# NVlabs/latentfusion

Hardware: AMD Instinct MI355X
Metric: pose-optim iters/sec (reconstruct+render+backward), 16 views, 128^3 voxels (higher is better)
Workload: dtype f32

## Files before the change

latentfusion_amd/csrc/build.py:

```python
import os
import subprocess
import sys

HERE = os.path.dirname(os.path.abspath(__file__))
SOURCES = ['resample.hip', 'splat.hip', 'conv.hip', 'pointwise.hip', 'image.hip', 'optim.hip', 'resize.hip', 'conv_split.hip', 'conv_wino.hip', 'wgrad.hip', 'sample2d.hip', 'gru.hip', 'wino_gemm.hip', 'reduce.hip', 'wino_fused.hip', 'conv_bf16.hip', 'occlusion.hip', 'conv_gru.hip', 'lift_mfma.hip', 'pw16.hip', 'wino_fused_f16x3.hip', 'wgrad_wide.hip', 'rows_gemm.hip', 'ibr.hip', 'latent.hip', 'points.hip', 'depth_init.hip', 'obs_prepare.hip', 'train_loss.hip', 'depth_points.hip', 'fps.hip']
LIB = os.path.join(HERE, 'liblf_hip.so')
EXTRA = {'conv_split.hip': ['-fno-slp-vectorize'], 'conv_gru.hip': ['-fno-slp-vectorize']}
FLAGS = ['--offload-arch=gfx950', '-O3', '-std=c++17', '-fPIC', '-fno-gpu-rdc', '-Wall', '-Wno-unused-function']


def _hipcc():
    for cand in (os.environ.get('HIPCC'), '/opt/rocm/bin/hipcc', 'hipcc'):
        if cand and (os.path.isabs(cand) and os.path.exists(cand) or not os.path.isabs(cand)):
            return cand
    raise RuntimeError('hipcc not found')


def needs_build():
    if not os.path.exists(LIB):
        return True
    t = os.path.getmtime(LIB)
    deps = [os.path.join(HERE, s) for s in SOURCES if os.path.exists(os.path.join(HERE, s))]
    deps += [os.path.join(HERE, f) for f in os.listdir(HERE) if f.endswith(('.h', '.inc'))]
    deps += [os.path.join(HERE, '..', '..', 'include', 'lf_hip.h'), os.path.join(HERE, '..', '..', 'include', 'lf_hip_experimental.h')]
    return any(os.path.getmtime(d) > t for d in deps)


def build(force=False, verbose=True):
    if not force and not needs_build():
        return LIB
    hipcc = _hipcc()
    objs = []
    procs = []
    for src in SOURCES:
        path = os.path.join(HERE, src)
        if not os.path.exists(path):
            continue
        obj = os.path.join(HERE, src.replace('.hip', '.o'))
        objs.append(obj)
        cmd = [hipcc, '-x', 'hip', '-c', path, '-o', obj] + FLAGS + EXTRA.get(src, [])
        procs.append((cmd, subprocess.Popen(cmd, stdout=subprocess.PIPE, stderr=subprocess.STDOUT)))
    for cmd, p in procs:
        out, _ = p.communicate()
        if p.returncode != 0:
            raise RuntimeError('hipcc failed: ' + ' '.join(cmd) + '\n' + out.decode())
        if verbose and out.strip():
            print(out.decode())
    cmd = [hipcc, '-shared', '-fPIC', '--offload-arch=gfx950', '-o', LIB] + objs
    r = subprocess.run(cmd, stdout=subprocess.PIPE, stderr=subprocess.STDOUT)
    if r.returncode != 0:
        raise RuntimeError('link failed:\n' + r.stdout.decode())
    if verbose:
        print('built', LIB)
    return LIB


if __name__ == '__main__':
    build(force='--force' in sys.argv)
```

latentfusion_amd/csrc/conv.hip:

```cpp
#include "lf_common.h"

namespace {

constexpr int TX = 16;

template <int DIMS> struct TileGeom;
template <> struct TileGeom<3> { static constexpr int TY = 4, TZ = 4, HY = 6, HZ = 6, TAPS = 27; };
template <> struct TileGeom<2> { static constexpr int TY = 16, TZ = 1, HY = 18, HZ = 1, TAPS = 9; };

template <int NT, int NR, bool WHOLE = false>
__device__ __forceinline__ void epilogue_store(f32x4 (&acc)[NT][NR], const long (&rowoff)[NR], const long (&rowidx)[NR],
                                               const float* __restrict__ bias, float* __restrict__ y,
                                               float* __restrict__ norm_out, int Cout, int co_base,
                                               int ysc, long yss, bool vec_out,
                                               float he, unsigned flags, float slope, float eps,
                                               const float* __restrict__ prev_y = nullptr,
                                               const float* __restrict__ prev_norm = nullptr, unsigned prev_flags = 0,
                                               float* __restrict__ amax_out = nullptr) {
  float lane_amax = 0.f;
  const int lane = threadIdx.x & 63;
  const int cq = lane >> 4;
  float bv[NT][4];
#pragma unroll
  for (int t = 0; t < NT; ++t)
// ... 619 lines not shown
  if (c16 <= 32) return 32;
  return (c16 + 63) & ~63;
}

extern "C" int lf_conv1x1_cout_padded(int Cout) {
  lf_clear_error();
  const int c16 = (Cout + 15) & ~15;
  if (c16 <= 16) return 16;
  if (c16 <= 32) return 32;
  if (c16 <= 64) return 64;
  return (c16 + 127) & ~127;
}

static int conv3x3_launch(const float* x, const float* wpack, const float* bias, float* y, float* norm_out,
                          int dims, int N, int D, int H, int W, int Cin, int Cout,
                          float he, unsigned flags, float slope, float eps, void* stream,
                          const float* prev_y, const float* prev_norm, unsigned prev_flags) {
  if (N <= 0 || D <= 0 || H <= 0 || W <= 0 || Cin <= 0 || Cout <= 0) return LF_EINVAL;
  if (prev_y != nullptr) {
    if (flags != 0 || bias != nullptr || (Cout != 16 && Cout != 32 && Cout != 64) || !lf_aligned16(prev_y)) return LF_EINVAL;
    if ((prev_flags & LF_EPI_PIXELNORM) && prev_norm == nullptr) return LF_EINVAL;
  }
  if (dims != 2 && dims != 3) return LF_EINVAL;
  if (dims == 2 && D != 1) return LF_EINVAL;
  if ((flags & LF_EPI_PIXELNORM) && Cout > 64) return LF_EINVAL;
  if (!lf_aligned16(x) || !lf_aligned16(y) || !lf_aligned16(wpack)) return LF_EALIGN;
  const int CinP = (Cin + 15) & ~15, CoutP = lf_conv3x3_cout_padded(Cout);
  const int ntiles = CoutP / 16;
  const int NT = ntiles >= 4 ? 4 : ntiles;
  const int groups = ntiles / NT;
  const int TY = dims == 3 ? 4 : 16, TZ = dims == 3 ? 4 : 1;
  const int tiles_x = (W + TX - 1) / TX, tiles_y = (H + TY - 1) / TY, tiles_z = (D + TZ - 1) / TZ;
  const long nblk = (long)tiles_x * tiles_y * tiles_z * N;
  if (nblk > 0x7fffffffL) return LF_EINVAL;
  dim3 grid((unsigned)nblk, groups), block(256);
  hipStream_t s = (hipStream_t)stream;
  if (Cin == 16 && Cout == 16 && dims == 3 && (long)D * H * W >= 4096 && (long)D * H * W * 64 < 0x7fffffffL &&
      slope > 0.f && slope < 1.f && (bias == nullptr || lf_aligned16(bias))) {
    const int ptx = (W + TX - 1) / TX, pty = (H + p3::TY - 1) / p3::TY, ptz = (D + p3::TZ - 1) / p3::TZ;
    const long pt = (long)ptx * pty * ptz * N;
    if (pt <= 0x7fffffffL) {
      const int cus = lf_cu_count();
      const unsigned pgrid = (unsigned)(pt < cus ? pt : cus);
      hipLaunchKernelGGL(conv3d_c16_persistent_kernel, dim3(pgrid), dim3(p3::NTHREADS), 0, s, x, wpack, bias, y, norm_out,
                         N, D, H, W, ptx, pty, ptz, (int)pt, he, flags, slope, eps, prev_y, prev_norm, prev_flags);
      return lf_launch_status();
    }
  }
  if (CinP == 16 && CoutP == 16) {
    if (dims == 3)
      hipLaunchKernelGGL((conv3x3_c16_kernel<3>), grid, block, 0, s, x, wpack, bias, y, norm_out, N, D, H, W, Cin, Cout,
                         tiles_x, tiles_y, tiles_z, he, flags, slope, eps, prev_y, prev_norm, prev_flags);
    else
      hipLaunchKernelGGL((conv3x3_c16_kernel<2>), grid, block, 0, s, x, wpack, bias, y, norm_out, N, D, H, W, Cin, Cout,
                         tiles_x, tiles_y, tiles_z, he, flags, slope, eps, prev_y, prev_norm, prev_flags);
    return lf_launch_status();
  }
#define LAUNCH(DM, T) hipLaunchKernelGGL((conv3x3_kernel<DM, T>), grid, block, 0, s, x, wpack, bias, y, norm_out, \
                                         N, D, H, W, Cin, Cout, CinP, CoutP, tiles_x, tiles_y, tiles_z, he, flags, slope, eps, \
                                         prev_y, prev_norm, prev_flags)
  if (dims == 3) { if (NT == 4) LAUNCH(3, 4); else if (NT == 2) LAUNCH(3, 2); else LAUNCH(3, 1); }
  else           { if (NT == 4) LAUNCH(2, 4); else if (NT == 2) LAUNCH(2, 2); else LAUNCH(2, 1); }
#undef LAUNCH
  return lf_launch_status();
}

extern "C" int lf_conv3x3_fwd(const float* x, const float* wpack, const float* bias, float* y, float* norm_out,
                              int dims, int N, int D, int H, int W, int Cin, int Cout,
                              float he, unsigned flags, float slope, float eps, void* stream) {
  lf_clear_error();
  return conv3x3_launch(x, wpack, bias, y, norm_out, dims, N, D, H, W, Cin, Cout, he, flags, slope, eps, stream,
                        nullptr, nullptr, 0);
}

extern "C" int lf_conv3x3_bwd_data(const float* gy, const float* wpack_t, float* gx, int dims, int N, int D, int H, int W,
                                   int Cin, int Cout, float he, const float* prev_y, const float* prev_norm,
                                   unsigned prev_flags, float slope, void* stream) {
  lf_clear_error();
  return conv3x3_launch(gy, wpack_t, nullptr, gx, nullptr, dims, N, D, H, W, Cin, Cout, he, 0, slope, 0.f, stream,
                        prev_y, prev_norm, prev_flags);
}

static int conv1x1_launch(const float* x, const float* wpack, const float* bias, float* y, float* norm_out,
                          int N, int P, int Cin, int ksl, long x_batch_stride, long x_slice_stride,
                          int Cout, long y_batch_stride, int y_row_stride, int y_slice_channels,
                          long y_slice_stride,
                          float he, unsigned flags, float slope, float eps, void* stream,
                          const float* prev_y, const float* prev_norm, unsigned prev_flags, float* amax_out = nullptr,
                          const float* xscale = nullptr) {
  if (N <= 0 || P <= 0 || Cin <= 0 || ksl <= 0 || Cout <= 0 || y_slice_channels <= 0) return LF_EINVAL;
  if (xscale != nullptr && (Cin & 3)) return LF_EALIGN;
  if (prev_y != nullptr) {
    if (flags != 0 || bias != nullptr || y_slice_channels != 16 || y_row_stride != 16 || (Cout & 15) ||
        !lf_aligned16(prev_y) || ((y_batch_stride | y_slice_stride) & 15))
      return LF_EINVAL;
    if ((prev_flags & LF_EPI_PIXELNORM) && prev_norm == nullptr) return LF_EINVAL;
    if ((prev_flags & LF_EPI_DOT) && (prev_flags != LF_EPI_DOT || prev_norm == nullptr)) return LF_EINVAL;
  }
  if (y_row_stride < (y_slice_channels < Cout ? y_slice_channels : Cout)) return LF_EINVAL;
  if (ksl > 1 && (Cin & 3)) return LF_EALIGN;
  if ((flags & LF_EPI_PIXELNORM) && Cout > 128) return LF_EINVAL;
  if (!lf_aligned16(x) || !lf_aligned16(y) || !lf_aligned16(wpack)) return LF_EALIGN;
  if (y == nullptr && !(prev_y != nullptr && (prev_flags & LF_EPI_DOT))) return LF_EINVAL;
  if ((Cin & 3) == 0 && ((x_batch_stride | x_slice_stride) & 3)) return LF_EALIGN;
  const int K = ksl * Cin, Kp = (K + 15) & ~15;
  const int CoutP = lf_conv1x1_cout_padded(Cout);
  const int ntiles = CoutP / 16;
  const int NT = ntiles >= 8 ? ((prev_y != nullptr && ntiles >= 16) ? 4 : 8) : ntiles;
  const int groups = ntiles / NT;
  dim3 grid((unsigned)((P + 63) / 64), groups, N), block(256);
  hipStream_t s = (hipStream_t)stream;
#define LAUNCH(T) hipLaunchKernelGGL((conv1x1_kernel<T>), grid, block, 0, s, x, wpack, bias, y, norm_out, \
                                     P, Cin, ksl, x_batch_stride, x_slice_stride, Cout, Kp, y_batch_stride, y_row_stride, \
                                     y_slice_channels, y_slice_stride, he, flags, slope, eps, prev_y, prev_norm, prev_flags, \
                                     amax_out, xscale)
  switch (NT) {
    case 1: LAUNCH(1); break;
    case 2: LAUNCH(2); break;
    case 4: LAUNCH(4); break;
    case 8: LAUNCH(8); break;
    default: return LF_EINVAL;
  }
#undef LAUNCH
  return lf_launch_status();
}

extern "C" int lf_conv1x1_fwd(const float* x, const float* wpack, const float* bias, float* y, float* norm_out,
                              int N, int P, int Cin, int ksl, long x_batch_stride, long x_slice_stride,
                              int Cout, long y_batch_stride, int y_row_stride, int y_slice_channels,
                              long y_slice_stride,
                              float he, unsigned flags, float slope, float eps, void* stream) {
  lf_clear_error();
  return conv1x1_launch(x, wpack, bias, y, norm_out, N, P, Cin, ksl, x_batch_stride, x_slice_stride, Cout,
                        y_batch_stride, y_row_stride, y_slice_channels, y_slice_stride, he, flags, slope, eps, stream,
                        nullptr, nullptr, 0);
}

extern "C" int lf_conv1x1_fwd_scaled(const float* x, const float* xscale, const float* wpack, const float* bias, float* y,
                                     float* norm_out, int N, int P, int Cin, int ksl, long x_batch_stride, long x_slice_stride,
                                     int Cout, long y_batch_stride, int y_row_stride, int y_slice_channels, long y_slice_stride,
                                     float he, unsigned flags, float slope, float eps, void* stream) {
  lf_clear_error();
  if (xscale == nullptr) return LF_EINVAL;
  return conv1x1_launch(x, wpack, bias, y, norm_out, N, P, Cin, ksl, x_batch_stride, x_slice_stride, Cout,
                        y_batch_stride, y_row_stride, y_slice_channels, y_slice_stride, he, flags, slope, eps, stream,
                        nullptr, nullptr, 0, nullptr, xscale);
}

extern "C" int lf_conv1x1_bwd_data(const float* gy, const float* wpack_t, float* gx, int N, int P, int Cin, int Cout,
                                   long y_batch_stride, int y_row_stride, int y_slice_channels, long y_slice_stride,
                                   float he, const float* prev_y, const float* prev_norm, unsigned prev_flags,
                                   float slope, float* amax_out, void* stream) {
  lf_clear_error();
  return conv1x1_launch(gy, wpack_t, nullptr, gx, nullptr, N, P, Cin, 1, (long)P * Cin, 0, Cout, y_batch_stride,
                        y_row_stride, y_slice_channels, y_slice_stride, he, 0, slope, 0.f, stream, prev_y, prev_norm,
                        prev_flags, amax_out);
}
```

latentfusion_amd/csrc/conv_wino.hip:

```cpp
#include "wino16_compute.h"

namespace {

template <bool SPLIT, int FUSE = 0, bool PACK = false, int FORM = WF_GENERIC, int OPT = 0, int ZST = 0>
__device__ __forceinline__ void conv3d_c16_wino_body(
    const float* __restrict__ x, const float* __restrict__ upack, const float* __restrict__ bias,
    float* __restrict__ y, float* __restrict__ norm_out,
    int N, int D, int H, int W, int tiles_x, int tiles_y, int tiles_z, int ntiles,
    float he, unsigned flags, float slope, float eps,
    const float* __restrict__ prev_y, const float* __restrict__ prev_norm, unsigned prev_flags,
    const float* __restrict__ amax_in, float* __restrict__ amax_out, const WinoProj pj = WinoProj()) {
  static_assert(FORM == WF_GENERIC || (!SPLIT && FUSE != 2 && PACK), "fixed forms: the packed all-fp32 kernels only");
  static_assert(OPT == 0 || OPT == 1, "");
  static_assert(FORM != WF_GENERIC || OPT == 0, "the generic kernel stays as it is");
  static_assert(ZST == 0 || (ZST == 1 && FORM != WF_GENERIC), "z-staged halo: the fixed forms only");
  constexpr bool HAS_BIAS = FORM == WF_FWD_BLOCK;
  if constexpr (FORM == WF_FWD_BLOCK) {
    flags = LF_EPI_LRELU | LF_EPI_PIXELNORM;
    prev_y = nullptr; prev_norm = nullptr; prev_flags = 0u; amax_out = nullptr;
  } else if constexpr (FORM == WF_DGRAD_PREV) {
    flags = 0u; prev_flags = LF_EPI_LRELU | LF_EPI_PIXELNORM;
    bias = nullptr; norm_out = nullptr; amax_out = nullptr;
  } else if constexpr (FORM == WF_DGRAD_PLAIN) {
    flags = 0u; prev_flags = 0u;
// ... 255 lines not shown
        v[k] = wino_epi_dgrad_plain(o[k], out_scale);
      } else if (prev_y == nullptr || addmode) {
        float ss = 0.f;
#pragma unroll
        for (int e = 0; e < 4; ++e) {
          float u = o[k][e] * out_scale + bv4[e];
          if (addmode) u += pyv[k][e];
          if (flags & LF_EPI_LRELU) u = fmaxf(u, u * slope);
          v[k][e] = u;
          ss += u * u;
        }
        if (flags & LF_EPI_PIXELNORM) {
          const float tq = quad_sum(ss) * (1.f / 16.f) + eps;
          const float rinv = fast_rsqrt(tq);
          rn[k] = tq * rinv;
          v[k] *= rinv;
        }
      }
    }
    TS(6);
    if constexpr (FUSE != 2) halo_commit();
    TS(7);
#pragma unroll
    for (int k = 0; k < 4; ++k) {
      if constexpr (FORM == WF_DGRAD_PREV) {
        if (!(WINO_ABL & 1)) v[k] = wino_epi_dgrad_prev(o[k], pyv[k], pnv[k], out_scale, slope);
      } else if (!(WINO_ABL & 1) && prev_y != nullptr && !addmode) {
        const f32x4 yp = pyv[k];
        v[k] = o[k] * out_scale;
        if (prev_flags & LF_EPI_PIXELNORM) {
          const float dot = quad_sum(v[k][0] * yp[0] + v[k][1] * yp[1] + v[k][2] * yp[2] + v[k][3] * yp[3]) * (1.f / 16.f);
          const float rinv = fast_rcp(pnv[k]);
#pragma unroll
          for (int e = 0; e < 4; ++e) v[k][e] = (v[k][e] - yp[e] * dot) * rinv;
        }
        if (prev_flags & LF_EPI_LRELU) {
#pragma unroll
          for (int e = 0; e < 4; ++e) v[k][e] = yp[e] > 0.f ? v[k][e] : v[k][e] * slope;
        }
      }
      if (okv[k]) {
        __builtin_nontemporal_store(v[k], (f32x4*)(ybase + (unsigned)(voxi[k] * 64)));
        if (!(WINO_ABL & 16) && (prev_y == nullptr || addmode) && (flags & LF_EPI_PIXELNORM) && (FORM == WF_FWD_BLOCK || nbase != nullptr) && eq == 0) nbase[voxi[k]] = rn[k];
        if (amax_out != nullptr)
          wave_amax = fmaxf(wave_amax, fmaxf(fmaxf(fabsf(v[k][0]), fabsf(v[k][1])), fmaxf(fabsf(v[k][2]), fabsf(v[k][3]))));
      }
    }
    if constexpr (FUSE == 2) {
#define WINO16_PROJBWD_NEXT
#include "wino16_projbwd.inc"
    }
    if constexpr (FUSE == 1) {
#define WINO16_PROJFWD_TILE
#include "wino16_projfwd.inc"
    }
    TS(8);
    lds_barrier();
    cx = nx; cy = ny; cz = nz; cn = nn;
    if constexpr (FUSE == 2) {
#define WINO16_PROJBWD_COLUMN
#include "wino16_projbwd.inc"
    }
  }
  if (amax_out != nullptr) {
    float m = wave_amax;
#pragma unroll
    for (int o2 = 32; o2 > 0; o2 >>= 1) m = fmaxf(m, __shfl_xor(m, o2, 64));
    lf_amax_publish(amax_out, m, lane);
  }
}

template <bool PACK>
__global__ void __launch_bounds__(256, 2) conv3d_c16_wino_kernel(
    const float* __restrict__ x, const float* __restrict__ upack, const float* __restrict__ bias,
    float* __restrict__ y, float* __restrict__ norm_out, int N, int D, int H, int W, int tiles_x, int tiles_y, int tiles_z,
    int ntiles, float he, unsigned flags, float slope, float eps, const float* __restrict__ prev_y,
    const float* __restrict__ prev_norm, unsigned prev_flags, float* __restrict__ amax_out) {
  conv3d_c16_wino_body<false, 0, PACK>(x, upack, bias, y, norm_out, N, D, H, W, tiles_x, tiles_y, tiles_z, ntiles, he, flags, slope, eps,
                              prev_y, prev_norm, prev_flags, nullptr, amax_out);
}

__global__ void __launch_bounds__(256, 2) conv3d_c16_wino_f16x3_kernel(
    const float* __restrict__ x, const float* __restrict__ upack, const float* __restrict__ bias,
    float* __restrict__ y, float* __restrict__ norm_out, int N, int D, int H, int W, int tiles_x, int tiles_y, int tiles_z,
    int ntiles, float he, unsigned flags, float slope, float eps, const float* __restrict__ prev_y,
    const float* __restrict__ prev_norm, unsigned prev_flags, const float* __restrict__ amax_in,
    float* __restrict__ amax_out) {
  conv3d_c16_wino_body<true>(x, upack, bias, y, norm_out, N, D, H, W, tiles_x, tiles_y, tiles_z, ntiles, he, flags, slope, eps,
                             prev_y, prev_norm, prev_flags, amax_in, amax_out);
}

template <bool PACK>
__global__ void __launch_bounds__(256, 2) conv3d_c16_wino_projfwd_kernel(
    const float* __restrict__ x, const float* __restrict__ upack, const float* __restrict__ bias,
    float* __restrict__ y, float* __restrict__ norm_out, int N, int D, int H, int W, int tiles_x, int tiles_y, int tiles_z,
    int ntiles, float he, unsigned flags, float slope, float eps, const float* __restrict__ prev_y,
    const float* __restrict__ prev_norm, unsigned prev_flags, WinoProj pj) {
  conv3d_c16_wino_body<false, 1, PACK>(x, upack, bias, y, norm_out, N, D, H, W, tiles_x, tiles_y, tiles_z, ntiles, he, flags, slope,
                                 eps, prev_y, prev_norm, prev_flags, nullptr, nullptr, pj);
}

template <bool PACK>
__global__ void __launch_bounds__(256, 2) conv3d_c16_wino_projbwd_kernel(
    const float* __restrict__ x, const float* __restrict__ upack, const float* __restrict__ bias,
    float* __restrict__ y, float* __restrict__ norm_out, int N, int D, int H, int W, int tiles_x, int tiles_y, int tiles_z,
    int ntiles, float he, unsigned flags, float slope, float eps, const float* __restrict__ prev_y,
    const float* __restrict__ prev_norm, unsigned prev_flags, WinoProj pj) {
  conv3d_c16_wino_body<false, 2, PACK>(x, upack, bias, y, norm_out, N, D, H, W, tiles_x, tiles_y, tiles_z, ntiles, he, flags, slope,
                                 eps, prev_y, prev_norm, prev_flags, nullptr, nullptr, pj);
}

template <int FORM, int OPT>
__global__ void __launch_bounds__(256, 2) conv3d_c16_wino_form_kernel(
    const float* __restrict__ x, const float* __restrict__ upack, const float* __restrict__ bias,
    float* __restrict__ y, float* __restrict__ norm_out, int N, int D, int H, int W, int tiles_x, int tiles_y, int tiles_z,
    int ntiles, float he, unsigned flags, float slope, float eps, const float* __restrict__ prev_y,
    const float* __restrict__ prev_norm, unsigned prev_flags, float* __restrict__ amax_out) {
  conv3d_c16_wino_body<false, 0, true, FORM, OPT>(x, upack, bias, y, norm_out, N, D, H, W, tiles_x, tiles_y, tiles_z, ntiles, he, flags,
                                                 slope, eps, prev_y, prev_norm, prev_flags, nullptr, amax_out);
}

template <int FORM, int OPT>
__global__ void __launch_bounds__(256, 2) conv3d_c16_wino_projfwd_form_kernel(
    const float* __restrict__ x, const float* __restrict__ upack, const float* __restrict__ bias,
    float* __restrict__ y, float* __restrict__ norm_out, int N, int D, int H, int W, int tiles_x, int tiles_y, int tiles_z,
    int ntiles, float he, unsigned flags, float slope, float eps, const float* __restrict__ prev_y,
    const float* __restrict__ prev_norm, unsigned prev_flags, WinoProj pj) {
  conv3d_c16_wino_body<false, 1, true, FORM, OPT>(x, upack, bias, y, norm_out, N, D, H, W, tiles_x, tiles_y, tiles_z, ntiles, he, flags,
                                                 slope, eps, prev_y, prev_norm, prev_flags, nullptr, nullptr, pj);
}

template <int FORM, int OPT>
__global__ void __launch_bounds__(256, 2) conv3d_c16_wino_zst_form_kernel(
    const float* __restrict__ x, const float* __restrict__ upack, const float* __restrict__ bias,
    float* __restrict__ y, float* __restrict__ norm_out, int N, int D, int H, int W, int tiles_x, int tiles_y, int tiles_z,
    int ntiles, float he, unsigned flags, float slope, float eps, const float* __restrict__ prev_y,
    const float* __restrict__ prev_norm, unsigned prev_flags, float* __restrict__ amax_out) {
  conv3d_c16_wino_body<false, 0, true, FORM, OPT, 1>(x, upack, bias, y, norm_out, N, D, H, W, tiles_x, tiles_y, tiles_z, ntiles, he, flags,
                                                    slope, eps, prev_y, prev_norm, prev_flags, nullptr, amax_out);
}

template <int FORM, int OPT>
__global__ void __launch_bounds__(256, 2) conv3d_c16_wino_projfwd_zst_form_kernel(
    const float* __restrict__ x, const float* __restrict__ upack, const float* __restrict__ bias,
    float* __restrict__ y, float* __restrict__ norm_out, int N, int D, int H, int W, int tiles_x, int tiles_y, int tiles_z,
    int ntiles, float he, unsigned flags, float slope, float eps, const float* __restrict__ prev_y,
    const float* __restrict__ prev_norm, unsigned prev_flags, WinoProj pj) {
  conv3d_c16_wino_body<false, 1, true, FORM, OPT, 1>(x, upack, bias, y, norm_out, N, D, H, W, tiles_x, tiles_y, tiles_z, ntiles, he, flags,
                                                    slope, eps, prev_y, prev_norm, prev_flags, nullptr, nullptr, pj);
}

int g_wino_pack = 1;
int g_wino_forms = 1;
constexpr bool wino_zst_default[4] = {true, false, false, true};
bool wino_zst(int idx) { return g_wino_forms == 4 || (g_wino_forms == 1 && wino_zst_default[idx]); }

int wino_form_of(const float* bias, const float* norm_out, unsigned flags, const float* prev_y, const float* prev_norm,
                 unsigned prev_flags, const float* amax_out) {
  const unsigned full = LF_EPI_LRELU | LF_EPI_PIXELNORM;
  if (!g_wino_pack || !g_wino_forms || amax_out != nullptr) return WF_GENERIC;
  if (flags == full && bias != nullptr && norm_out != nullptr && prev_y == nullptr) return WF_FWD_BLOCK;
  if (flags == 0u && bias == nullptr && prev_y != nullptr && prev_norm != nullptr && prev_flags == full) return WF_DGRAD_PREV;
  if (flags == 0u && bias == nullptr && prev_y == nullptr) return WF_DGRAD_PLAIN;
  return WF_GENERIC;
}

template <auto kernel, bool COLUMNS = false, typename... Extra>
int launch_wino(const float* x, const void* upack, const float* bias, float* y, float* norm_out, int N, int D,
                int H, int W, float he, unsigned flags, float slope, float eps, const float* prev_y, const float* prev_norm,
                unsigned prev_flags, void* stream, Extra... extra) {
  if (N <= 0 || D <= 0 || H <= 0 || W <= 0) return LF_EINVAL;
  if ((long)D * H * W * 64 >= 0x7fffffffL || !(slope > 0.f && slope < 1.f)) return LF_EINVAL;
  if (!lf_aligned16(x) || !lf_aligned16(y) || !lf_aligned16(upack) || (bias && !lf_aligned16(bias))) return LF_EALIGN;
  const bool add = prev_y != nullptr && (prev_flags & LF_EPI_ADD);
  if (add && prev_flags != LF_EPI_ADD) return LF_EINVAL;
  if (prev_y != nullptr && !add && (flags != 0 || bias != nullptr)) return LF_EINVAL;
  if ((prev_flags & LF_EPI_PIXELNORM) && prev_y != nullptr && prev_norm == nullptr) return LF_EINVAL;
  const int ptx = (W + TXw - 1) / TXw, pty = (H + TYw - 1) / TYw, ptz = (D + TZw - 1) / TZw;
  const long pt = (long)ptx * pty * ptz * N;
  if (pt > 0x7fffffffL) return LF_EINVAL;
  const int cus = lf_cu_count();
  const size_t shmem = (size_t)LDSw;
  static lf_devmask_t attr_set;
  {
    hipError_t e = lf_ensure_dyn_lds(attr_set, (const void*)kernel, (int)shmem);
    if (e != hipSuccess) return (int)e;
  }
  const long want = 2L * cus;
  const long units = COLUMNS ? pt / ptz : pt;
  const unsigned grid = (unsigned)(units < want ? units : want);
  hipLaunchKernelGGL(kernel, dim3(grid), dim3(256), shmem, (hipStream_t)stream, x, (const float*)upack, bias, y, norm_out, N, D,
                     H, W, ptx, pty, ptz, (int)pt, he, flags, slope, eps, prev_y, prev_norm, prev_flags, extra...);
  return lf_launch_status();
}

}

int lf_internal_wino_set_pack(int v) {
  const int prev = g_wino_pack;
  if (v == 0 || v == 1) g_wino_pack = v;
  return prev;
}
int lf_internal_wino_set_forms(int v) {
  const int prev = g_wino_forms;
  if (v >= 0 && v <= 4) g_wino_forms = v;
  return prev;
}

extern "C" size_t lf_conv3d_c16_wino_upack_floats(void) { return (size_t)4 * 16 * 4 * 64; }

extern "C" int lf_conv3d_c16_wino(const float* x, const float* upack, const float* bias, float* y, float* norm_out,
                                  int N, int D, int H, int W, float he, unsigned flags, float slope, float eps,
                                  const float* prev_y, const float* prev_norm, unsigned prev_flags,
                                  float* amax_out, void* stream) {
  lf_clear_error();
#define LF_WINO_FORM(F, O) \
  launch_wino<conv3d_c16_wino_form_kernel<F, O>>(x, upack, bias, y, norm_out, N, D, H, W, he, flags, slope, eps, prev_y, prev_norm, \
                                                 prev_flags, stream, amax_out)
#define LF_WINO_ZST(F) \
  launch_wino<conv3d_c16_wino_zst_form_kernel<F, 1>>(x, upack, bias, y, norm_out, N, D, H, W, he, flags, slope, eps, prev_y, prev_norm, \
                                                     prev_flags, stream, amax_out)
#define LF_WINO_OPTS(F) (g_wino_forms == 2 ? LF_WINO_FORM(F, 0) : wino_zst(F - WF_FWD_BLOCK) ? LF_WINO_ZST(F) : LF_WINO_FORM(F, 1))
  switch (wino_form_of(bias, norm_out, flags, prev_y, prev_norm, prev_flags, amax_out)) {
    case WF_FWD_BLOCK: return LF_WINO_OPTS(WF_FWD_BLOCK);
    case WF_DGRAD_PREV: return LF_WINO_OPTS(WF_DGRAD_PREV);
    case WF_DGRAD_PLAIN: return LF_WINO_OPTS(WF_DGRAD_PLAIN);
    default: break;
  }
#undef LF_WINO_OPTS
#undef LF_WINO_ZST
#undef LF_WINO_FORM
  return g_wino_pack ? launch_wino<conv3d_c16_wino_kernel<true>>(x, upack, bias, y, norm_out, N, D, H, W, he, flags, slope, eps, prev_y,
                                                                  prev_norm, prev_flags, stream, amax_out)
                     : launch_wino<conv3d_c16_wino_kernel<false>>(x, upack, bias, y, norm_out, N, D, H, W, he, flags, slope, eps, prev_y,
                                                                   prev_norm, prev_flags, stream, amax_out);
}

extern "C" size_t lf_conv3d_c16_wino_split_upack_halfs(void) { return (size_t)4 * 16 * 2 * 64 * 4; }

extern "C" int lf_conv3d_c16_wino_split(const float* x, const void* upack, const float* bias, float* y, float* norm_out,
                                        int N, int D, int H, int W, float he, unsigned flags, float slope, float eps,
                                        const float* prev_y, const float* prev_norm, unsigned prev_flags,
                                        const float* amax_in, float* amax_out, void* stream) {
  lf_clear_error();
  return launch_wino<conv3d_c16_wino_f16x3_kernel>(x, upack, bias, y, norm_out, N, D, H, W, he, flags, slope, eps, prev_y,
                     prev_norm, prev_flags, stream, amax_in, amax_out);
}

extern "C" size_t lf_conv3d_c16_wino_proj_pack_floats(int D) { return (size_t)(D > 0 ? D : 0) * 64 * 4; }

extern "C" int lf_conv3d_c16_wino_projfwd(const float* x, const float* upack, const float* bias, float* y, float* norm_out,
                                          int N, int D, int H, int W, float he, unsigned flags, float slope, float eps,
                                          const float* proj_wA, const float* proj_bias, float* zp, float* pnorm,
                                          float proj_he, unsigned proj_flags, void* stream) {
  lf_clear_error();
  if (proj_wA == nullptr || zp == nullptr) return LF_EINVAL;
  if (!lf_aligned16(proj_wA) || !lf_aligned16(zp) || (proj_bias && !lf_aligned16(proj_bias))) return LF_EALIGN;
  if ((proj_flags & ~(LF_EPI_LRELU | LF_EPI_PIXELNORM)) != 0) return LF_EINVAL;
  WinoProj pj = {proj_wA, proj_bias, zp, pnorm, nullptr, nullptr, proj_he, proj_flags};
  if (wino_form_of(bias, norm_out, flags, nullptr, nullptr, 0u, nullptr) == WF_FWD_BLOCK) {
#define LF_WINO_FORM(O) \
  launch_wino<conv3d_c16_wino_projfwd_form_kernel<WF_FWD_BLOCK, O>, true>(x, upack, bias, y, norm_out, N, D, H, W, he, flags, slope, eps, \
                                                                          nullptr, nullptr, 0u, stream, pj)
    if (g_wino_forms != 2 && wino_zst(3))
      return launch_wino<conv3d_c16_wino_projfwd_zst_form_kernel<WF_FWD_BLOCK, 1>, true>(x, upack, bias, y, norm_out, N, D, H, W, he, flags,
                                                                                         slope, eps, nullptr, nullptr, 0u, stream, pj);
    return g_wino_forms == 2 ? LF_WINO_FORM(0) : LF_WINO_FORM(1);
#undef LF_WINO_FORM
  }
  return g_wino_pack ? launch_wino<conv3d_c16_wino_projfwd_kernel<true>, true>(x, upack, bias, y, norm_out, N, D, H, W, he, flags, slope,
                                                                                eps, nullptr, nullptr, 0u, stream, pj)
                     : launch_wino<conv3d_c16_wino_projfwd_kernel<false>, true>(x, upack, bias, y, norm_out, N, D, H, W, he, flags, slope,
                                                                                 eps, nullptr, nullptr, 0u, stream, pj);
}

extern "C" int lf_conv3d_c16_wino_projbwd(const float* gp, const float* proj_wtA, float proj_he, const float* act,
                                          const float* act_norm, unsigned act_flags, const float* upack, float* y,
                                          int N, int D, int H, int W, float he, float slope, const float* prev_y,
                                          const float* prev_norm, unsigned prev_flags, void* stream) {
  lf_clear_error();
  if (gp == nullptr || proj_wtA == nullptr || act == nullptr) return LF_EINVAL;
  if ((act_flags & LF_EPI_PIXELNORM) && act_norm == nullptr) return LF_EINVAL;
  if ((act_flags & ~(LF_EPI_LRELU | LF_EPI_PIXELNORM)) != 0) return LF_EINVAL;
  if (!lf_aligned16(gp) || !lf_aligned16(proj_wtA) || (prev_y && !lf_aligned16(prev_y))) return LF_EALIGN;
  if (prev_y != nullptr && (prev_flags & LF_EPI_ADD)) return LF_EINVAL;
  WinoProj pj = {proj_wtA, nullptr, nullptr, nullptr, gp, act_norm, proj_he, act_flags};
  return g_wino_pack ? launch_wino<conv3d_c16_wino_projbwd_kernel<true>, true>(act, upack, nullptr, y, nullptr, N, D, H, W, he, 0u, slope,
                                                                                0.f, prev_y, prev_norm, prev_flags, stream, pj)
                     : launch_wino<conv3d_c16_wino_projbwd_kernel<false>, true>(act, upack, nullptr, y, nullptr, N, D, H, W, he, 0u, slope,
                                                                                 0.f, prev_y, prev_norm, prev_flags, stream, pj);
}
```

latentfusion_amd/csrc/lf_common.h:

```cpp
#pragma once
#include <hip/hip_runtime.h>
#include <stdint.h>
#include "../../include/lf_hip.h"
#include "../../include/lf_hip_experimental.h"

#define LF_WAVE 64

typedef float f32x4 __attribute__((ext_vector_type(4)));

static inline void lf_clear_error() { (void)hipGetLastError(); }

static inline int lf_launch_status() {
  hipError_t e = hipGetLastError();
  return (int)e;
}

static inline bool lf_aligned16(const void* p) { return (((uintptr_t)p) & 15u) == 0; }

#include <atomic>
typedef std::atomic<unsigned long long> lf_devmask_t;
static inline hipError_t lf_ensure_dyn_lds(lf_devmask_t& done, const void* fn, int bytes) {
  int dev = 0;
  if (hipGetDevice(&dev) != hipSuccess) dev = 0;
  const unsigned long long bit = 1ull << (dev & 63);
  if (done.load(std::memory_order_acquire) & bit) return hipSuccess;
  const hipError_t e = hipFuncSetAttribute(fn, hipFuncAttributeMaxDynamicSharedMemorySize, bytes);
  if (e == hipSuccess) done.fetch_or(bit, std::memory_order_release);
  return e;
}

static inline int lf_cu_count() {
  static std::atomic<int> cus[64];
  int dev = 0, v = 0;
  const bool known = hipGetDevice(&dev) == hipSuccess;
  std::atomic<int>& slot = cus[dev & 63];
  const int c = slot.load(std::memory_order_relaxed);
  if (c != 0) return c;
  const int n = (known && hipDeviceGetAttribute(&v, hipDeviceAttributeMultiprocessorCount, dev) == hipSuccess && v > 0) ? v : 256;
  slot.store(n, std::memory_order_relaxed);
  return n;
}

__device__ __forceinline__ float lf_wave_sum(float v) {
#pragma unroll
  for (int o = 32; o > 0; o >>= 1) v += __shfl_xor(v, o, 64);
  return v;
}

#define LF_AMAX_SLOTS 64
#define LF_AMAX_STRIDE 32
static_assert(LF_AMAX_FLOATS == LF_AMAX_SLOTS * LF_AMAX_STRIDE, "lf_hip.h: LF_AMAX_FLOATS");

__device__ __forceinline__ void lf_amax_publish(float* base, float wave_max, int lane) {
  if (lane == 0 && wave_max > 0.f)
    atomicMax((unsigned int*)(base + (blockIdx.x % LF_AMAX_SLOTS) * LF_AMAX_STRIDE), __float_as_uint(wave_max));
}

__device__ __forceinline__ float lf_amax_read(const float* base, int lane) {
  float m = base[(lane % LF_AMAX_SLOTS) * LF_AMAX_STRIDE];
#pragma unroll
  for (int o = 32; o > 0; o >>= 1) m = fmaxf(m, __shfl_xor(m, o, 64));
  return m;
}

__device__ __forceinline__ float lf_lrelu(float v, float slope) { return v > 0.f ? v : v * slope; }

int lf_internal_ring_bf16_set_wgs(int v);
int lf_internal_wino_set_pack(int v);
int lf_internal_wino_set_forms(int v);
int lf_internal_fused_set_cfg(int v);
int lf_internal_splat_set_variant(int v);
int lf_internal_splat_set_chunk_cap(int v);
```

latentfusion_amd/csrc/resample.hip:

```cpp
#include "resample_map.h"

namespace {

typedef unsigned u32x4_t __attribute__((ext_vector_type(4)));

struct Tap {
  int x0, y0, z0, x1, y1, z1;
  float tx, ty, tz;
  float mx, my, mz;
};

__device__ __forceinline__ float lattice01(int i, int size, float step) {
  return (i < max(size / 2, 1)) ? step * (float)i : 1.f - step * (float)(size - 1 - i);
}


template <int KIND>
__device__ __forceinline__ void eval_grid(const float* __restrict__ cf, int x, int y, int z,
                                          int W, int H, int D, Steps st, float& gx, float& gy, float& gz,
                                          float& a, float& b, float& k) {
  a = lattice01(x, W, st.w);
  b = lattice01(y, H, st.h);
  k = lattice01(z, D, st.d);
  if (KIND == LF_MAP_O2C) {
// ... 363 lines not shown
  if (int e = lf_launch_status()) return e;
  hipLaunchKernelGGL(resample_bwd_coef_reduce, dim3(N), dim3(256), 0, s, partial, nblk, gcoef);
  return lf_launch_status();
}

static int bwd_coef_launch(const float* gout, const float* vol, int vol_n, const float* coef,
                           float* gcoef, void* scratch, size_t scratch_bytes,
                           int N, int part_n, int D, int H, int W, int C, void* stream) {
  if (N <= 0 || D <= 0 || H <= 0 || W <= 0 || C <= 0) return LF_EINVAL;
  if (vol_n != 1 && vol_n != N) return LF_EINVAL;
  BwdCoefPlan p;
  if (int e = bwd_coef_plan(gout, vol, scratch_bytes, N, part_n, D, H, W, C, p)) return e;
  const long bstride = vol_n == 1 ? 0 : p.nvox * C;
  hipStream_t s = (hipStream_t)stream;
  float* partial = (float*)scratch;
  if (g_resample_variant == 4 && p.vec && C == 16 && p.nvox * 64 < 0xffffffffL && W <= 65535) {
    const int ntx = (W + LT_X - 1) / LT_X, nty = (H + LT_Y - 1) / LT_Y, ntz = (D + LT_Z - 1) / LT_Z;
    const long nb = staged_bwd_blocks(D, H, W);
    if (nb * N > 0x7fffffffL) return LF_EINVAL;
    hipLaunchKernelGGL((resample_bwd_coef_staged_kernel<STAGED_TPW>), dim3((unsigned)(nb * N)), dim3(256), 0, s, gout, vol, bstride, coef,
                       partial, (int)nb, D, H, W, ntx, nty, ntz, p.st);
    return bwd_coef_finish(partial, (int)nb, gcoef, N, s);
  }
  if (g_resample_variant >= 2 && p.vec && C == 16 && p.vpb >= 64 && p.nvox * 64 < 0xffffffffL) {
    const int v = g_bwd_coef_variant;
    const bool big = p.vpb >= 256;
#define LAUNCH(...) hipLaunchKernelGGL((__VA_ARGS__), p.grid, dim3(256), 0, s, gout, vol, bstride, coef, partial, p.nblk, p.vpb, p.bt, D, H, W, p.st)
    if (v == 1)              LAUNCH(resample_bwd_coef_c16_kernel<1, 1>);
    else if (v == 2)         LAUNCH(resample_bwd_coef_c16_kernel<1, 2>);
    else if (v == 3)         LAUNCH(resample_bwd_coef_c16_kernel<4, 2>);
    else if (v == 6 && big)  LAUNCH(resample_bwd_coef_c16_dedup_kernel<2, 1>);
    else if (v == 7 && big)  LAUNCH(resample_bwd_coef_c16_dedup_kernel<1, 1>);
    else if (v == 8 && big)  LAUNCH(resample_bwd_coef_c16_dedup_kernel<2, 4>);
    else if (v == 9 && big)  LAUNCH(resample_bwd_coef_c16_dedup_kernel<1, 5>);
    else if (v == 10 && big) LAUNCH(resample_bwd_coef_c16_dedup_kernel<2, 1, true>);
    else if (v == 11 && big) LAUNCH(resample_bwd_coef_c16_dedup_kernel<1, 1, true>);
    else if (v == 4)         LAUNCH(resample_bwd_coef_c16_kernel<6, 1>);
    else                     LAUNCH(resample_bwd_coef_c16_kernel<8, 1>);
#undef LAUNCH
  } else if (p.vec) {
    hipLaunchKernelGGL((resample_bwd_coef_kernel<4>), p.grid, dim3(256), 0, s, gout, vol, bstride, coef, partial, p.nblk, p.vpb, p.bt, N, D, H, W, C, p.lpv, p.st);
  } else {
    hipLaunchKernelGGL((resample_bwd_coef_kernel<1>), p.grid, dim3(256), 0, s, gout, vol, bstride, coef, partial, p.nblk, p.vpb, p.bt, N, D, H, W, C, p.lpv, p.st);
  }
  return bwd_coef_finish(partial, p.nblk, gcoef, N, s);
}

extern "C" int lf_resample3d_bwd_coef(const float* gout, const float* vol, int vol_n, const float* coef,
                                      float* gcoef, void* scratch, size_t scratch_bytes,
                                      int N, int D, int H, int W, int C, void* stream) {
  lf_clear_error();
  return bwd_coef_launch(gout, vol, vol_n, coef, gcoef, scratch, scratch_bytes, N, N, D, H, W, C, stream);
}

extern "C" int lf_resample3d_bwd_coef_part(const float* gout, const float* vol, int vol_n, const float* coef,
                                           float* gcoef, void* scratch, size_t scratch_bytes,
                                           int N, int D, int H, int W, int C, int part_n, void* stream) {
  lf_clear_error();
  if (!gout || !vol || !coef || !gcoef || !scratch) return LF_EINVAL;
  if (part_n <= 0 || N <= 0) return LF_EINVAL;
  return bwd_coef_launch(gout, vol, vol_n, coef, gcoef, scratch, scratch_bytes, N, part_n, D, H, W, C, stream);
}

extern "C" int lf_resample3d_fwd_indexed(const float* vol, int vol_n, const int* vol_idx, const float* coef, int kind, float* out,
                                         int N, int D, int H, int W, int C, void* stream) {
  lf_clear_error();
  if (!vol || !vol_idx || !coef || !out) return LF_EINVAL;
  if (N <= 0 || D <= 0 || H <= 0 || W <= 0 || C <= 0 || vol_n < 1) return LF_EINVAL;
  if (kind != LF_MAP_O2C && kind != LF_MAP_C2O) return LF_EINVAL;
  if (((uintptr_t)vol_idx & 3) != 0) return LF_EALIGN;
  const long bstride = (long)D * H * W * C;
  FwdPlan p;
  if (int e = fwd_plan(vol, out, N, D, H, W, C, p)) return e;
  hipStream_t s = (hipStream_t)stream;
  if (g_resample_variant >= 3 && p.vec && C == 16 && (long)D * H * W * 64 < 0xffffffffL) {
    LAUNCH_BY_KIND(resample_fwd_c16_indexed_kernel, p.grid, vol, bstride, vol_idx, vol_n, coef, out, D, H, W, p.nbz, p.st);
  } else if (g_resample_variant >= 2 && p.vec && (long)D * H * W * C * 4 < 0xffffffffL) {
    LAUNCH_BY_KIND(resample_fwd_lean_indexed_kernel, p.grid, vol, bstride, vol_idx, vol_n, coef, out, D, H, W, C, p.lpt, p.tlx, p.tly, p.tlz, p.nbz, p.st);
  } else {
#define LAUNCH(K, V) hipLaunchKernelGGL((resample_fwd_indexed_kernel<K, V>), p.grid, dim3(256), 0, s, vol, bstride, vol_idx, vol_n, coef, out, N, D, H, W, C, p.lpt, p.tlx, p.tly, p.tlz, p.nbz, p.st)
    if (kind == LF_MAP_O2C) { if (p.vec) LAUNCH(LF_MAP_O2C, 4); else LAUNCH(LF_MAP_O2C, 1); }
    else                    { if (p.vec) LAUNCH(LF_MAP_C2O, 4); else LAUNCH(LF_MAP_C2O, 1); }
#undef LAUNCH
  }
  return lf_launch_status();
}

extern "C" size_t lf_resample3d_bwd_coef_indexed_scratch_bytes(int N, int part_n, int D, int H, int W) {
  if (N <= 0 || part_n <= 0) return 0;
  return bwd_coef_scratch_bytes(N, part_n, D, H, W);
}

extern "C" int lf_resample3d_bwd_coef_indexed(const float* gout, const float* vol, int vol_n, const int* vol_idx, const float* coef,
                                              float* gcoef, void* scratch, size_t scratch_bytes,
                                              int N, int D, int H, int W, int C, int part_n, void* stream) {
  lf_clear_error();
  if (!gout || !vol || !vol_idx || !coef || !gcoef || !scratch) return LF_EINVAL;
  if (part_n <= 0 || N <= 0 || vol_n < 1) return LF_EINVAL;
  if (D <= 0 || H <= 0 || W <= 0 || C <= 0) return LF_EINVAL;
  if (((uintptr_t)vol_idx & 3) != 0) return LF_EALIGN;
  BwdCoefPlan p;
  if (int e = bwd_coef_plan(gout, vol, scratch_bytes, N, part_n, D, H, W, C, p)) return e;
  const long bstride = p.nvox * C;
  hipStream_t s = (hipStream_t)stream;
  float* partial = (float*)scratch;
  if (g_resample_variant >= 2 && p.vec && C == 16 && p.vpb >= 64 && p.nvox * 64 < 0xffffffffL) {
    if (p.vpb >= 256)
      hipLaunchKernelGGL((resample_bwd_coef_c16_dedup_indexed_kernel<2, 1, true>), p.grid, dim3(256), 0, s, gout, vol, bstride, vol_idx, vol_n, coef, partial, p.nblk, p.vpb, p.bt, D, H, W, p.st);
    else
      hipLaunchKernelGGL((resample_bwd_coef_c16_indexed_kernel<8, 1>), p.grid, dim3(256), 0, s, gout, vol, bstride, vol_idx, vol_n, coef, partial, p.nblk, p.vpb, p.bt, D, H, W, p.st);
  } else if (p.vec) {
    hipLaunchKernelGGL((resample_bwd_coef_indexed_kernel<4>), p.grid, dim3(256), 0, s, gout, vol, bstride, vol_idx, vol_n, coef, partial, p.nblk, p.vpb, p.bt, N, D, H, W, C, p.lpv, p.st);
  } else {
    hipLaunchKernelGGL((resample_bwd_coef_indexed_kernel<1>), p.grid, dim3(256), 0, s, gout, vol, bstride, vol_idx, vol_n, coef, partial, p.nblk, p.vpb, p.bt, N, D, H, W, C, p.lpv, p.st);
  }
  return bwd_coef_finish(partial, p.nblk, gcoef, N, s);
}

extern "C" int lf_resample3d_bwd_vol(const float* gout, const float* coef, int kind, float* gvol, int vol_n,
                                     int N, int D, int H, int W, int C, void* stream) {
  lf_clear_error();
  if (N <= 0 || D <= 0 || H <= 0 || W <= 0 || C <= 0) return LF_EINVAL;
  if (vol_n != 1 && vol_n != N) return LF_EINVAL;
  const long bstride = vol_n == 1 ? 0 : (long)D * H * W * C;
  const long items = (long)D * H * W * C;
  dim3 grid((unsigned)min((items + 255) / 256, (long)65535 * 16), N), block(256);
  hipStream_t s = (hipStream_t)stream;
  if (kind == LF_MAP_O2C)
    hipLaunchKernelGGL((resample_bwd_vol_kernel<LF_MAP_O2C>), grid, block, 0, s, gout, coef, gvol, bstride, N, D, H, W, C, make_steps(D, H, W));
  else if (kind == LF_MAP_C2O)
    hipLaunchKernelGGL((resample_bwd_vol_kernel<LF_MAP_C2O>), grid, block, 0, s, gout, coef, gvol, bstride, N, D, H, W, C, make_steps(D, H, W));
  else
    return LF_EINVAL;
  return lf_launch_status();
}

#ifdef STAGE_TS
extern "C" int lf_debug_stage_ts(void* dst) {
  return (int)hipMemcpyFromSymbol(dst, HIP_SYMBOL(g_stage_ts), sizeof(unsigned long long) * 256 * 16, 0, hipMemcpyDeviceToHost);
}
#endif

extern "C" int lf_set_tuning(int key, int value) {
  if (key == 1) {
    const int prev = g_resample_variant;
    if (value >= 1 && value <= 5) g_resample_variant = value;
    return prev;
  }
  if (key == 4) return lf_internal_splat_set_variant(value);
  if (key == 6) return lf_internal_splat_set_chunk_cap(value);
  if (key == 3) return lf_internal_fused_set_cfg(value);
  if (key == 7) return lf_internal_wino_set_pack(value);
  if (key == 8) return lf_internal_wino_set_forms(value);
  if (key == 5) return lf_internal_ring_bf16_set_wgs(value);
  if (key == 2) {
    const int prev = g_bwd_coef_variant;
    if (value >= 1 && value <= 11) g_bwd_coef_variant = value;
    return prev;
  }
  return LF_EINVAL;
}

extern "C" int lf_resample3d_fwd_io(const void* vol, int vol_n, const float* coef, int kind, void* out,
                                    int N, int D, int H, int W, int io, void* stream) {
  lf_clear_error();
  if (N <= 0 || D <= 0 || H <= 0 || W <= 0 || io < 0 || io > 3) return LF_EINVAL;
  if ((vol_n != 1 && vol_n != N) || (kind != LF_MAP_O2C && kind != LF_MAP_C2O)) return LF_EINVAL;
  if (!lf_aligned16(vol) || !lf_aligned16(out)) return LF_EALIGN;
  if ((long)D * H * W * 64 >= 0xffffffffL) return LF_EINVAL;
  const long bstride = vol_n == 1 ? 0 : (long)D * H * W * 16;
  const int nbz4 = (D + 3) >> 2;
  if ((long)nbz4 * N > 65535 || ((H + 3) >> 2) > 65535) return LF_EINVAL;
  dim3 g4((unsigned)((W + 3) >> 2), (unsigned)((H + 3) >> 2), (unsigned)(nbz4 * N)), block(256);
  const Steps st = make_steps(D, H, W);
  typedef void (*kern_t)(const float*, long, const float*, float*, int, int, int, int, Steps);
  static const kern_t kerns[2][4] = {
      {resample_fwd_c16_kernel<LF_MAP_O2C, 0>, resample_fwd_c16_kernel<LF_MAP_O2C, 1>, resample_fwd_c16_kernel<LF_MAP_O2C, 2>, resample_fwd_c16_kernel<LF_MAP_O2C, 3>},
      {resample_fwd_c16_kernel<LF_MAP_C2O, 0>, resample_fwd_c16_kernel<LF_MAP_C2O, 1>, resample_fwd_c16_kernel<LF_MAP_C2O, 2>, resample_fwd_c16_kernel<LF_MAP_C2O, 3>}};
  hipLaunchKernelGGL(kerns[kind == LF_MAP_O2C ? 0 : 1][io], g4, block, 0, (hipStream_t)stream, (const float*)vol, bstride, coef, (float*)out, D, H, W, nbz4, st);
  return lf_launch_status();
}
```

Before: 198.7.

## Add streaming MFMA kernel for 16-channel 1x1 conv backward-data with fused epilogue

Adds a dedicated persistent kernel for the 1x1 conv data-gradient when Cin is 16 and the previous layer used leaky-ReLU plus pixel-norm. The kernel computes each 16-channel output slice with a 16x16x4 MFMA and fuses the pixel-norm and leaky-ReLU backward into the same pass. It software-pipelines the loads across slices and writes with nontemporal stores. It also enables the z-staged halo for every fixed Winograd form, not just two of them. The new path is gated by shape checks and a tuning key, with the generic conv1x1 launch kept as the fallback.

```diff
diff --git a/latentfusion_amd/csrc/build.py b/latentfusion_amd/csrc/build.py
--- a/latentfusion_amd/csrc/build.py
+++ b/latentfusion_amd/csrc/build.py
@@ -3,7 +3,7 @@
 import sys
 
 HERE = os.path.dirname(os.path.abspath(__file__))
-SOURCES = ['resample.hip', 'splat.hip', 'conv.hip', 'pointwise.hip', 'image.hip', 'optim.hip', 'resize.hip', 'conv_split.hip', 'conv_wino.hip', 'wgrad.hip', 'sample2d.hip', 'gru.hip', 'wino_gemm.hip', 'reduce.hip', 'wino_fused.hip', 'conv_bf16.hip', 'occlusion.hip', 'conv_gru.hip', 'lift_mfma.hip', 'pw16.hip', 'wino_fused_f16x3.hip', 'wgrad_wide.hip', 'rows_gemm.hip', 'ibr.hip', 'latent.hip', 'points.hip', 'depth_init.hip', 'obs_prepare.hip', 'train_loss.hip', 'depth_points.hip', 'fps.hip']
+SOURCES = ['resample.hip', 'splat.hip', 'conv.hip', 'pointwise.hip', 'image.hip', 'optim.hip', 'resize.hip', 'conv_split.hip', 'conv_wino.hip', 'wgrad.hip', 'sample2d.hip', 'gru.hip', 'wino_gemm.hip', 'reduce.hip', 'wino_fused.hip', 'conv_bf16.hip', 'occlusion.hip', 'conv_gru.hip', 'lift_mfma.hip', 'pw16.hip', 'wino_fused_f16x3.hip', 'wgrad_wide.hip', 'rows_gemm.hip', 'ibr.hip', 'latent.hip', 'points.hip', 'depth_init.hip', 'obs_prepare.hip', 'train_loss.hip', 'depth_points.hip', 'fps.hip', 'proj_bwd_c16.hip']
 LIB = os.path.join(HERE, 'liblf_hip.so')
 EXTRA = {'conv_split.hip': ['-fno-slp-vectorize'], 'conv_gru.hip': ['-fno-slp-vectorize']}
 FLAGS = ['--offload-arch=gfx950', '-O3', '-std=c++17', '-fPIC', '-fno-gpu-rdc', '-Wall', '-Wno-unused-function']
diff --git a/latentfusion_amd/csrc/conv.hip b/latentfusion_amd/csrc/conv.hip
--- a/latentfusion_amd/csrc/conv.hip
+++ b/latentfusion_amd/csrc/conv.hip
@@ -795,6 +795,10 @@
                                    float he, const float* prev_y, const float* prev_norm, unsigned prev_flags,
                                    float slope, float* amax_out, void* stream) {
   lf_clear_error();
+  int status = 0;
+  if (lf_internal_proj_bwd_c16(gy, wpack_t, gx, N, P, Cin, Cout, y_batch_stride, y_row_stride, y_slice_channels, y_slice_stride,
+                               he, prev_y, prev_norm, prev_flags, slope, amax_out, stream, &status))
+    return status;
   return conv1x1_launch(gy, wpack_t, nullptr, gx, nullptr, N, P, Cin, 1, (long)P * Cin, 0, Cout, y_batch_stride,
                         y_row_stride, y_slice_channels, y_slice_stride, he, 0, slope, 0.f, stream, prev_y, prev_norm,
                         prev_flags, amax_out);
diff --git a/latentfusion_amd/csrc/conv_wino.hip b/latentfusion_amd/csrc/conv_wino.hip
--- a/latentfusion_amd/csrc/conv_wino.hip
+++ b/latentfusion_amd/csrc/conv_wino.hip
@@ -431,7 +431,7 @@
 
 int g_wino_pack = 1;
 int g_wino_forms = 1;
-constexpr bool wino_zst_default[4] = {true, false, false, true};
+constexpr bool wino_zst_default[4] = {true, true, true, true};
 bool wino_zst(int idx) { return g_wino_forms == 4 || (g_wino_forms == 1 && wino_zst_default[idx]); }
 
 int wino_form_of(const float* bias, const float* norm_out, unsigned flags, const float* prev_y, const float* prev_norm,
diff --git a/latentfusion_amd/csrc/lf_common.h b/latentfusion_amd/csrc/lf_common.h
--- a/latentfusion_amd/csrc/lf_common.h
+++ b/latentfusion_amd/csrc/lf_common.h
@@ -69,5 +69,10 @@
 int lf_internal_wino_set_pack(int v);
 int lf_internal_wino_set_forms(int v);
 int lf_internal_fused_set_cfg(int v);
+int lf_internal_proj_bwd_set_stream(int v);
+bool lf_internal_proj_bwd_c16(const float* gy, const float* wpack_t, float* gx, int N, int P, int Cin, int Cout,
+                              long y_batch_stride, int y_row_stride, int y_slice_channels, long y_slice_stride, float he,
+                              const float* prev_y, const float* prev_norm, unsigned prev_flags, float slope,
+                              const float* amax_out, void* stream, int* status);
 int lf_internal_splat_set_variant(int v);
 int lf_internal_splat_set_chunk_cap(int v);
diff --git a/latentfusion_amd/csrc/proj_bwd_c16.hip b/latentfusion_amd/csrc/proj_bwd_c16.hip
--- /dev/null
+++ b/latentfusion_amd/csrc/proj_bwd_c16.hip
@@ -0,0 +1,140 @@
+#include "lf_common.h"
+
+#ifndef PROJ_BWD_WGS
+#define PROJ_BWD_WGS 8
+#endif
+#ifndef PROJ_BWD_PF
+#define PROJ_BWD_PF 4
+#endif
+#ifndef PROJ_BWD_NT
+#define PROJ_BWD_NT 1
+#endif
+
+namespace {
+
+__device__ __forceinline__ f32x4 proj_epi_prev(const f32x4 acc, const f32x4 yp, float pn, float he, float slope) {
+#pragma clang fp contract(off)
+  f32x4 v;
+#pragma unroll
+  for (int e = 0; e < 4; ++e) v[e] = __builtin_fmaf(he, acc[e], 0.f);
+  float dot = __builtin_fmaf(v[3], yp[3], __builtin_fmaf(v[2], yp[2], __builtin_fmaf(v[0], yp[0], v[1] * yp[1])));
+  dot = dot + __shfl_xor(dot, 16, 64);
+  dot = dot + __shfl_xor(dot, 32, 64);
+  dot = dot * (1.f / 16.f);
+  const float rinv = 1.0f / pn;
+#pragma unroll
+  for (int e = 0; e < 4; ++e) {
+    const float g = rinv * __builtin_fmaf(-yp[e], dot, v[e]);
+    v[e] = yp[e] > 0.f ? g : slope * g;
+  }
+  return v;
+}
+
+template <int PF, bool NTS>
+__global__ void __launch_bounds__(256) proj_bwd_c16_stream_kernel(
+    const float* __restrict__ gp, const float* __restrict__ wt, float* __restrict__ g, const float* __restrict__ act,
+    const float* __restrict__ norm, int P, int D, long batch_stride, int runs_per_sample, int nruns, float he, float slope) {
+  const int lane = threadIdx.x & 63, wave = threadIdx.x >> 6;
+  const int li = lane & 15, cq = lane >> 4;
+  const long slice = (long)P * 16;
+  for (int run = blockIdx.x; run < nruns; run += gridDim.x) {
+    const int n = run / runs_per_sample;
+    const int p = (run - n * runs_per_sample) * 64 + wave * 16 + li;
+    const bool live = p < P;
+    const long rec = (long)n * batch_stride + (long)(live ? p : 0) * 16 + cq * 4;
+    const float* arow = wt + li * 16 + cq * 4;
+    f32x4 b = (f32x4){0.f, 0.f, 0.f, 0.f};
+#ifndef PROJ_BWD_ABL
+    b = *(const f32x4*)(gp + ((long)n * P + (live ? p : 0)) * 16 + cq * 4);
+#endif
+    f32x4 av[PF], yv[PF];
+    float nv[PF];
+    auto request = [&](int u, int d) {
+#ifndef PROJ_BWD_ABL
+      av[u] = *(const f32x4*)(arow + (long)d * 256);
+#endif
+      const long off = rec + d * slice;
+      yv[u] = *(const f32x4*)(act + off);
+      nv[u] = norm[off >> 4];
+    };
+    auto step = [&](int u, int d, bool all_live) {
+      const f32x4 yp = yv[u];
+      const float pn = nv[u];
+#ifdef PROJ_BWD_ABL
+      f32x4 out = yp;
+      out[3] = pn;
+#else
+      const f32x4 a = av[u];
+      f32x4 acc = (f32x4){0.f, 0.f, 0.f, 0.f};
+#pragma unroll
+      for (int st = 0; st < 4; ++st) acc = __builtin_amdgcn_mfma_f32_16x16x4f32(a[st], b[st], acc, 0, 0, 0);
+      const f32x4 out = proj_epi_prev(acc, yp, pn, he, slope);
+#endif
+      if (all_live || live) {
+        f32x4* dst = (f32x4*)(g + rec + d * slice);
+        if (NTS) __builtin_nontemporal_store(out, dst);
+        else *dst = out;
+      }
+    };
+    const int wave_p0 = __builtin_amdgcn_readfirstlane(p - li);
+    if (wave_p0 + 16 <= P && D % PF == 0) {
+#pragma unroll
+      for (int u = 0; u < PF; ++u) request(u, u);
+      for (int d0 = 0; d0 < D - PF; d0 += PF) {
+#pragma unroll
+        for (int u = 0; u < PF; ++u) {
+          step(u, d0 + u, true);
+          request(u, d0 + u + PF);
+          __builtin_amdgcn_sched_barrier(0);
+        }
+      }
+#pragma unroll
+      for (int u = 0; u < PF; ++u) step(u, D - PF + u, true);
+    } else {
+#pragma unroll
+      for (int u = 0; u < PF; ++u)
+        if (u < D) request(u, u);
+      for (int d0 = 0; d0 < D; d0 += PF) {
+#pragma unroll
+        for (int u = 0; u < PF; ++u) {
+          const int d = d0 + u;
+          if (d >= D) break;
+          step(u, d, false);
+          if (d + PF < D) request(u, d + PF);
+        }
+      }
+    }
+  }
+}
+
+int g_proj_bwd_stream = 1;
+
+}
+
+int lf_internal_proj_bwd_set_stream(int v) {
+  const int prev = g_proj_bwd_stream;
+  if (v == 0 || v == 1) g_proj_bwd_stream = v;
+  return prev;
+}
+
+bool lf_internal_proj_bwd_c16(const float* gy, const float* wpack_t, float* gx, int N, int P, int Cin, int Cout,
+                              long y_batch_stride, int y_row_stride, int y_slice_channels, long y_slice_stride, float he,
+                              const float* prev_y, const float* prev_norm, unsigned prev_flags, float slope,
+                              const float* amax_out, void* stream, int* status) {
+  if (!g_proj_bwd_stream) return false;
+  if (N <= 0 || P <= 0 || Cin != 16 || y_slice_channels != 16 || y_row_stride != 16) return false;
+  if (Cout < 16 || (Cout & 15) || y_slice_stride != (long)P * 16 || (y_batch_stride & 15) || y_batch_stride < 0) return false;
+  if (gy == nullptr || wpack_t == nullptr || gx == nullptr || prev_y == nullptr || prev_norm == nullptr) return false;
+  if (prev_flags != (LF_EPI_LRELU | LF_EPI_PIXELNORM) || amax_out != nullptr) return false;
+  if (!lf_aligned16(gy) || !lf_aligned16(wpack_t) || !lf_aligned16(gx) || !lf_aligned16(prev_y) || !lf_aligned16(prev_norm))
+    return false;
+  const int D = Cout >> 4;
+  const long rps = ((long)P + 63) / 64, nruns = rps * N;
+  if (nruns > 0x7fffffffL) return false;
+  const long want = (long)PROJ_BWD_WGS * lf_cu_count();
+  const unsigned grid = (unsigned)(nruns < want ? nruns : want);
+  hipLaunchKernelGGL((proj_bwd_c16_stream_kernel<PROJ_BWD_PF, PROJ_BWD_NT != 0>), dim3(grid), dim3(256), 0, (hipStream_t)stream,
+                     gy, wpack_t, gx, prev_y, prev_norm, P, D, y_batch_stride, (int)rps, (int)nruns, he, slope);
+  *status = lf_launch_status();
+  return true;
+}
diff --git a/latentfusion_amd/csrc/resample.hip b/latentfusion_amd/csrc/resample.hip
--- a/latentfusion_amd/csrc/resample.hip
+++ b/latentfusion_amd/csrc/resample.hip
@@ -539,6 +539,7 @@
   if (key == 3) return lf_internal_fused_set_cfg(value);
   if (key == 7) return lf_internal_wino_set_pack(value);
   if (key == 8) return lf_internal_wino_set_forms(value);
+  if (key == 9) return lf_internal_proj_bwd_set_stream(value);
   if (key == 5) return lf_internal_ring_bf16_set_wgs(value);
   if (key == 2) {
     const int prev = g_bwd_coef_variant;
```

Result: no change. 200.0 (median of 6 runs) (+0.7%).
